# sumitsk/algp

Hardware: AMD Instinct MI355X
Metric: GP-fit+MI-score throughput (N train x M candidates) (higher is better)
Workload: dtype f64

## Files before the change

### algp_amd/csrc/api.hip

```cpp
#include "api_impl.h"

using namespace algp;

namespace algp {

int fail(algp_ctx* c, int code, const std::string& msg) {
    if (c) c->err = msg;
    return code;
}

int ensure(algp_ctx* c, DevBuf& b, size_t bytes) {
    if (bytes <= b.cap && b.p) return ALGP_OK;
    if (bytes == 0) bytes = 256;
    if (b.p) {
        hipStreamSynchronize(c->stream);
        hipFree(b.p);
        c->dev_bytes -= (int64_t)b.cap;
        b.p = nullptr;
        b.cap = 0;
    }
    const size_t want = (bytes + 255) / 256 * 256;
    hipError_t e = hipMalloc(&b.p, want);
    if (e != hipSuccess) {
        b.p = nullptr;
// ... 437 lines not shown

template struct Impl<float>;
template struct Impl<double>;

}

extern "C" {

int algp_version(void) { return 100; }

int algp_device_count(void) {
    int n = 0;
    if (hipGetDeviceCount(&n) != hipSuccess) { (void)hipGetLastError(); return 0; }
    return n;
}

int algp_create(int device_id, int dtype, algp_ctx** out) {
    if (!out || (dtype != ALGP_F32 && dtype != ALGP_F64)) return ALGP_ERR_BAD_ARG;
    *out = nullptr;
    setenv("GPU_MAX_HW_QUEUES", "8", 0);
    int n = 0;
    if (hipGetDeviceCount(&n) != hipSuccess || n <= 0) { (void)hipGetLastError(); return ALGP_ERR_NO_DEVICE; }
    if (device_id < 0 || device_id >= n) return ALGP_ERR_BAD_ARG;
    if (hipSetDevice(device_id) != hipSuccess) return ALGP_ERR_HIP;
    algp_ctx* c = new algp_ctx();
    c->device = device_id;
    c->dtype = dtype;
    c->es = dtype == ALGP_F64 ? 8 : 4;
    if (hipStreamCreateWithFlags(&c->stream, hipStreamNonBlocking) != hipSuccess) { delete c; return ALGP_ERR_HIP; }
    if (hipStreamCreateWithFlags(&c->stream2, hipStreamNonBlocking) != hipSuccess) { hipStreamDestroy(c->stream); delete c; return ALGP_ERR_HIP; }
    if (hipStreamCreateWithFlags(&c->stream3, hipStreamNonBlocking) != hipSuccess) c->stream3 = nullptr;
    if (hipStreamCreateWithFlags(&c->stream4, hipStreamNonBlocking) != hipSuccess) c->stream4 = nullptr;
    c->trsm_chunks = env_int("ALGP_TRSM_CHUNKS", c->trsm_chunks);
    c->cur = c->stream;
    if (ensure(c, c->scal, sizeof(double) * SC_COUNT) != ALGP_OK) { hipStreamDestroy(c->stream); delete c; return ALGP_ERR_OOM; }
    hipMemsetAsync(c->scal.p, 0, sizeof(double) * SC_COUNT, c->stream);
    hipStreamSynchronize(c->stream);
    *out = c;
    return ALGP_OK;
}

void algp_destroy(algp_ctx* c) {
    if (!c) return;
    hipSetDevice(c->device);
    hipStreamSynchronize(c->stream);
    prof_collect(c);
    DevBuf* bufs[] = {&c->Xs, &c->Xraw, &c->Cp, &c->Aidx, &c->yA, &c->varA, &c->y0, &c->L, &c->invD, &c->z, &c->alpha,
                      &c->scal, &c->Cidx, &c->ckind, &c->cextra, &c->Vt, &c->dstat, &c->mu, &c->alive, &c->scores,
                      &c->lrow, &c->remote, &c->commbuf, &c->tvec, &c->amax, &c->prevrows, &c->fresh, &c->lazypicks, &c->yraw, &c->uvec, &c->wvec, &c->acc3, &c->rowstat, &c->inv512, &c->inv512_scr, &c->trsm_tmp, &c->splitk, &c->dag_state, &c->dag_stats, &c->trsv_ctrl, &c->auxA, &c->auxInv, &c->auxW, &c->auxIdx,
                      &c->auxVar, &c->auxD, &c->hostStage, &c->rowx, &c->tailE, &c->tailPart, &c->ldpart};
    for (DevBuf* b : bufs) release(c, *b);
    release(c, c->mi);
    release(c, c->vr);
    dag_release(c);
    comm_destroy(c);
    for (hipEvent_t e : c->event_pool) hipEventDestroy(e);
    for (hipEvent_t e : c->sync_events) hipEventDestroy(e);
    hipStreamSynchronize(c->stream2);
    hipStreamDestroy(c->stream2);
    if (c->stream3) { hipStreamSynchronize(c->stream3); hipStreamDestroy(c->stream3); }
    if (c->stream4) { hipStreamSynchronize(c->stream4); hipStreamDestroy(c->stream4); }
    hipStreamDestroy(c->stream);
    delete c;
}

const char* algp_last_error(const algp_ctx* c) { return c ? c->err.c_str() : "null context"; }

int64_t algp_last_pivot(const algp_ctx* c) { return c ? c->pivot : 0; }

double algp_last_jitter(const algp_ctx* c) { return c ? c->last_jitter : 0.0; }

int algp_dtype(const algp_ctx* c) { return c ? c->dtype : -1; }

int algp_set_hypers(algp_ctx* c, int kernel, int D, const double* log_ls, double log_os, double log_noise) {
    CHECK_CTX(c);
    if (D < 1 || D > MAXD || !log_ls) return fail(c, ALGP_ERR_BAD_ARG, "set_hypers: 1 <= D <= 8 required");
    if (kernel != ALGP_KERNEL_RBF && kernel != ALGP_KERNEL_MATERN15) return fail(c, ALGP_ERR_BAD_ARG, "set_hypers: unknown kernel");
    if (c->hyp.set && c->hyp.D != D && c->n_pool > 0 && !c->pool_is_cov) {
        c->n_pool = 0;
        c->N = 0;
        c->pos_in_train.clear();
    }
// ... 50 lines not shown
    if (N < 0 || (N > 0 && (!idx || !y))) return fail(c, ALGP_ERR_BAD_ARG, "set_train: bad arguments");
    for (int64_t i = 0; i < N; ++i)
        if (idx[i] < 0 || idx[i] >= c->n_pool) return fail(c, ALGP_ERR_BAD_ARG, "set_train: index outside the pool");
    FINISH(c, DISPATCH(c, set_train(c, idx, N, y, var)));
}

int algp_set_constant_mean(algp_ctx* c, int enable, double value) {
    CHECK_CTX(c);
    if (enable && !(value == value)) return fail(c, ALGP_ERR_BAD_ARG, "set_constant_mean: NaN");
    c->mean_override = enable != 0;
    c->mean_value = value;
    return ALGP_OK;
}

#if ALGP_TEST_HOOKS
int64_t algp_debug_counter(algp_ctx* c, int which) {
    if (!c) return -1;
    switch (which) {
        case 0: return c->n_syncs;
        case 1: return c->factor_rows_from_vt;
        case 2: return c->rows_from_peers;
        case 3: return c->row_exchanges;
        case 4: return c->row_fallbacks;
        default: return -1;
    }
}
#endif

#if ALGP_TEST_HOOKS
int algp_debug_set_trsm_chunks(algp_ctx* c, int chunks) {
    CHECK_CTX(c);
    if (chunks < 0 || chunks > 4) return fail(c, ALGP_ERR_BAD_ARG, "debug_set_trsm_chunks: 0 (default) .. 4");
    hipStreamSynchronize(c->stream);
    if (chunks == 0) chunks = env_int("ALGP_TRSM_CHUNKS", 3);
    c->trsm_chunks = chunks;
    return ALGP_OK;
}
#endif

#if ALGP_TEST_HOOKS
int algp_debug_trsv_stall(algp_ctx* c, int block) {
    CHECK_CTX(c);
    if (block < -1) return fail(c, ALGP_ERR_BAD_ARG, "debug_trsv_stall: a block >= 0, or -1 to disarm");
    c->debug_trsv_stall_block = block;
    return ALGP_OK;
}
#endif

#if ALGP_TEST_HOOKS
int algp_debug_dag_stall(algp_ctx* c, int ticket) {
    CHECK_CTX(c);
    if (ticket < -1) return fail(c, ALGP_ERR_BAD_ARG, "debug_dag_stall: a ticket >= 0, or -1 to disarm");
    c->debug_dag_stall_ticket = ticket;
    return ALGP_OK;
}
#endif

int algp_entropy_from_cov(algp_ctx* c, const void* cov, int64_t k, double* H) {
    CHECK_CTX(c);
    if (k < 0 || !H || (k > 0 && !cov)) return fail(c, ALGP_ERR_BAD_ARG, "entropy_from_cov: bad arguments");
    FINISH(c, DISPATCH(c, entropy_from_cov(c, cov, k, H, nullptr, nullptr)));
}

int algp_set_entropy(algp_ctx* c, const int64_t* idx, int64_t m, const void* var, double* H) {
    CHECK_CTX(c);
    NEED_HYPERS(c);
// ... 103 lines not shown
```

### algp_amd/csrc/common.h

```cpp
#pragma once
#include <stdlib.h>
#include <hip/hip_runtime.h>
#include <stdint.h>
#include <string>
#include <vector>
#include "../../include/algp_hip.h"

namespace algp {

constexpr int NB = 128;
constexpr int MAXD = 8;
constexpr int MAX_APPEND = 128;
constexpr double ENT_CONST = 1.4189385332046727;

inline int64_t round_up(int64_t v, int64_t m) { return (v + m - 1) / m * m; }

constexpr int SC_LOGDET = 0;
constexpr int SC_INFO = 1;
constexpr int SC_AUXLOGDET = 2;
constexpr int SC_AUXINFO = 3;
constexpr int SC_AMAXV = 4;
constexpr int SC_AMAXI = 5;
constexpr int SC_PROBE = 6;
constexpr int SC_COMMIT = 8;
// ... 91 lines not shown

namespace algp {
__device__ __forceinline__ float kexp(float x) { return expf(x); }
__device__ __forceinline__ double kexp(double x) {
    const double k = __builtin_rint(x * 1.4426950408889634074);
    double r = __builtin_fma(-k, 6.93147180369123816490e-01, x);
    r = __builtin_fma(-k, 1.90821492927058770002e-10, r);
    double p = 1.6059043836821614599e-10;
    p = __builtin_fma(p, r, 2.0876756987868098979e-09);
    p = __builtin_fma(p, r, 2.5052108385441718775e-08);
    p = __builtin_fma(p, r, 2.7557319223985890653e-07);
    p = __builtin_fma(p, r, 2.7557319223985892511e-06);
    p = __builtin_fma(p, r, 2.4801587301587301566e-05);
    p = __builtin_fma(p, r, 1.9841269841269841253e-04);
    p = __builtin_fma(p, r, 1.3888888888888889419e-03);
    p = __builtin_fma(p, r, 8.3333333333333332177e-03);
    p = __builtin_fma(p, r, 4.1666666666666664354e-02);
    p = __builtin_fma(p, r, 1.6666666666666665741e-01);
    p = __builtin_fma(p, r, 0.5);
    p = __builtin_fma(p, r, 1.0);
    p = __builtin_fma(p, r, 1.0);
    return __builtin_ldexp(p, (int)k);
}
}

struct algp_ctx {
    int device = 0;
    int dtype = ALGP_F64;
    size_t es = 8;
    hipStream_t stream = nullptr;
    hipStream_t stream2 = nullptr;
    hipStream_t stream3 = nullptr, stream4 = nullptr;
    int trsm_chunks = 3;
    hipStream_t cur = nullptr;
    std::vector<hipEvent_t> sync_events;
    std::string err;
    int64_t pivot = 0;
    double last_jitter = 0;
    algp::Hypers hyp;

    int64_t n_pool = 0;
    bool pool_is_cov = false;
    algp::DevBuf Xs;
    algp::DevBuf Xraw;
    algp::DevBuf Cp;
    std::vector<int64_t> pos_in_train;
    std::vector<uint64_t> site_hash;

    int64_t N = 0, Npad = 0;
    int64_t Lld = 0;
    int64_t Nfact = 0;
    std::vector<int64_t> fact_idx;
    std::vector<double> fact_var;
    std::vector<double> train_var_host;
    uint64_t fact_hyp_stamp = 0, hyp_stamp = 1;
    bool train_dirty = false;
    int64_t kept_rows_last = 0;
    std::vector<int64_t> train_idx;
    bool mean_override = false;
    double mean_value = 0;
    bool train_has_repeats = false;
    algp::DevBuf Aidx, yA, varA, y0, L, invD, z, alpha, scal;
    double ybar = 0, logdet = 0, yalpha = 0;
    bool factored = false;
    algp::DevBuf yraw, uvec, wvec;
    std::vector<double> train_y_host, fact_y;
    int64_t uw_rows = 0;
    int64_t uw_stable = 0;
    algp::DevBuf acc3;
    algp::DevBuf rowstat;
    algp::DevBuf splitk;
    algp::DevBuf ldpart;
    algp::DevBuf tailPart;
    algp::DevBuf tailE;
    algp::DevBuf inv512, inv512_scr, trsm_tmp;
    std::vector<algp::DagCache> dag_cache;
    algp::DevBuf dag_state;
    algp::DevBuf trsv_ctrl;
    algp::DevBuf dag_stats;
    int64_t acc_cols = 0, acc_M = -1;
    int64_t factor_rows_from_vt = 0;
    bool alpha_valid = false;

    int64_t M = 0, Mpad = 0, ldv = 0;
    int64_t ncols = 0;
    int prior_noise = 1;
    std::vector<int64_t> cand_idx;
    std::vector<int64_t> cand_pos;
    algp::DevBuf Cidx, ckind, cextra, Vt, dstat, mu, alive, scores, lrow, tvec, amax;
    std::vector<algp::PickRec> picks;
    algp::DevBuf prevrows;
    algp::DevBuf remote;
    algp::DevBuf fresh, lazypicks;
    bool lazy_stale = false;
    bool bounds_valid = false;
    double lazy_ss = 0, lazy_delta = 0;
    bool solved = false;
    int64_t ldv_cap = 0;
    std::vector<int64_t> vt_fact_idx, vt_cand_idx;
    std::vector<double> vt_fact_var;
    std::vector<int> vt_kind;
    uint64_t vt_hyp_stamp = 0;
    int vt_prior_noise = -1;
    bool vt_has_extra = false;
    int64_t kept_cols_last = 0;

    algp::MiState mi;
// ... 187 lines not shown
```

### algp_amd/csrc/gemm.hip

```cpp
#include "common.h"
#include <hip/hip_ext.h>
#include "mfma.h"
#include <algorithm>
#include <type_traits>
#include <stdio.h>
#include <stdlib.h>

namespace algp {

template <typename T>
struct GemmArgs {
    const T* A;
    const T* B;
    const T* C;
    T* D;
    int64_t lda, ldb, ldc, ldd;
    int64_t sA, sB, sC, sD;
    int tiles_m, tiles_n, ktiles;
    T alpha, beta;
    int lower_only;
    int ktri;
    int kcut;
    const T* stat_w;
    T* stat_out;
    int64_t stat_ld;
};

typedef __attribute__((address_space(3))) void* lds_vp;
typedef const __attribute__((address_space(1))) void* glb_vp;

template <int CTRL>
__device__ __forceinline__ float dpp_row(float x) {
    return __int_as_float(__builtin_amdgcn_update_dpp(0, __float_as_int(x), CTRL, 0xf, 0xf, false));
}
template <int CTRL>
__device__ __forceinline__ double dpp_row(double x) {
    const int lo = __builtin_amdgcn_update_dpp(0, __double2loint(x), CTRL, 0xf, 0xf, false);
    const int hi = __builtin_amdgcn_update_dpp(0, __double2hiint(x), CTRL, 0xf, 0xf, false);
    return __hiloint2double(hi, lo);
}
template <typename T>
__device__ __forceinline__ T row16_sum(T x) {
    x += dpp_row<0x128>(x);
    x += dpp_row<0x124>(x);
    x += dpp_row<0x122>(x);
    x += dpp_row<0x121>(x);
    return x;
}

template <typename T>
struct VrGemmArgs : GemmArgs<T> {
    const int64_t* cidx;
    const int* ckind;
    int64_t M;
    int64_t ncol0;
    const T* Xs;
    const T* Cp;
    int64_t n_pool;
// ... 46 lines not shown
                const int col = wc * 64 + j * 16 + fr;
                const int64_t pcol = pc[col];
                T cv;
                if (g.Cp) {
                    cv = g.Cp[prow * g.n_pool + pcol];
                } else {
                    T r2 = (T)0;
#pragma unroll
                    for (int d = 0; d < MAXD; ++d) {
                        const T df = xrow[d] - xc[col * MAXD + d];
                        r2 += df * df;
                    }
                    if (g.kernel == ALGP_KERNEL_RBF) cv = g.os * kexp((T)-0.5 * r2);
                    else {
                        const T rr = sqrt(r2) * (T)1.7320508075688772;
                        cv = g.os * ((T)1 + rr) * kexp(-rr);
                    }
                    if (prow == pcol) cv += g.noise;
                }
                T e = kap * cv - acc[i][j][r];
                e = mc[col] ? e : (T)0;
                s2 += e * e;
            }
            s2 = row16_sum<T>(s2);
            if (fr == 0) red[wc * 128 + row] = s2;
        }
    __syncthreads();
    if (tid < 128) g.stat_out[(int64_t)bn * g.stat_ld + m0 + tid] = red[tid] + red[128 + tid];
}

#ifndef ALGP_GEMM_XOR_MASK
#define ALGP_GEMM_XOR_MASK 2
#endif
template <typename T, bool STATS = false, typename Args = GemmArgs<T>>
__global__ __launch_bounds__(256, 2) void gemm_nt_kernel_dma4(Args g) {
    constexpr bool VR = !std::is_same<Args, GemmArgs<T>>::value;
    static_assert(!(VR && STATS), "one epilogue per kernel");
    constexpr int NST = 4;
    using F = MF<T>;
    using acc_t = typename F::acc_t;
    using chunk_t = typename F::chunk_t;
    constexpr int EPC = F::EPC;
    constexpr int BK = 4 * EPC;

    __shared__ __attribute__((aligned(1024))) char smem[NST * 16384];

    const int nwg = gridDim.x;
    int bm, bn;
    if (g.ktri) {
        int local = blockIdx.x >> 3;
        bm = blockIdx.x & 7;
        while (bm < g.tiles_m && local > bm) { local -= bm + 1; bm += 8; }
        if (bm >= g.tiles_m) return;
        bn = local;
    } else {
        int sid;
        {
            const int id = blockIdx.x, xcd = id & 7, q = nwg >> 3, r = nwg & 7;
            sid = (xcd < r ? xcd * (q + 1) : r * (q + 1) + (xcd - r) * q) + (id >> 3);
        }
        if (g.lower_only) {
            bm = (int)((sqrt(8.0 * (double)sid + 1.0) - 1.0) * 0.5);
            while ((int64_t)(bm + 1) * (bm + 2) / 2 <= sid) ++bm;
            while ((int64_t)bm * (bm + 1) / 2 > sid) --bm;
            bn = sid - (int)((int64_t)bm * (bm + 1) / 2);
        } else {
            bm = sid / g.tiles_n;
            bn = sid - bm * g.tiles_n;
        }
    }
    const int64_t m0 = (int64_t)bm * 128, n0 = (int64_t)bn * 128;
    const int kskip = g.ktri ? bm * (128 / (4 * MF<T>::EPC)) : 0;
    const int tid = threadIdx.x, lane = tid & 63;
    const int wave = __builtin_amdgcn_readfirstlane(tid >> 6);
    const int wr = wave >> 1, wc = wave & 1;
    const int64_t bz = blockIdx.y;

    const int srow = lane >> 2;
    const int schunk = (lane & 3) ^ ((lane >> 4) & ALGP_GEMM_XOR_MASK);
    const T* Ag = g.A + bz * g.sA + (m0 + 32 * wave + srow) * g.lda + schunk * EPC + (int64_t)kskip * BK;
    const T* Bg = g.B + bz * g.sB + (n0 + 32 * wave + srow) * g.ldb + schunk * EPC + (int64_t)kskip * BK;
    auto stage = [&](int st, int kt) {
        char* As = smem + st * 16384 + wave * 2048;
        char* Bs = As + 8192;
#pragma unroll
        for (int i = 0; i < 2; ++i) {
            __builtin_amdgcn_global_load_lds((glb_vp)(Ag + (int64_t)(16 * i) * g.lda + (int64_t)kt * BK),
                                             (lds_vp)(As + i * 1024), 16, 0, 0);
            __builtin_amdgcn_global_load_lds((glb_vp)(Bg + (int64_t)(16 * i) * g.ldb + (int64_t)kt * BK),
                                             (lds_vp)(Bs + i * 1024), 16, 0, 0);
        }
    };

    const int fr = lane & 15, fg = lane >> 4;
    const int coff = ((fg ^ ((fr >> 2) & ALGP_GEMM_XOR_MASK)) << 4);
    const int aoff = (wr * 64 + fr) * 64 + coff;
    const int boff = (wc * 64 + fr) * 64 + coff;

    acc_t acc[4][4];
#pragma unroll
    for (int i = 0; i < 4; ++i)
#pragma unroll
        for (int j = 0; j < 4; ++j)
#pragma unroll
            for (int r = 0; r < 4; ++r) acc[i][j][r] = (T)0;

    int nkt = g.ktiles * 2 - kskip;
    if (g.kcut && (bn + 1) * (128 / BK) < nkt) nkt = (bn + 1) * (128 / BK);
#pragma unroll
    for (int t = 0; t < NST - 1; ++t)
        if (t < nkt) stage(t, t);

    auto fread = [&](int st, chunk_t (&a)[4], chunk_t (&b)[4]) {
        const char* As = smem + st * 16384;
        const char* Bs = As + 8192;
#pragma unroll
        for (int t = 0; t < 4; ++t) a[t] = *reinterpret_cast<const chunk_t*>(As + aoff + t * 1024);
#pragma unroll
        for (int t = 0; t < 4; ++t) b[t] = *reinterpret_cast<const chunk_t*>(Bs + boff + t * 1024);
    };
    auto fmac = [&](const chunk_t (&a)[4], const chunk_t (&b)[4]) {
#pragma unroll
        for (int j = 0; j < 4; ++j)
#pragma unroll
            for (int e = 0; e < EPC; ++e)
#pragma unroll
                for (int i = 0; i < 4; ++i) acc[i][j] = F::mfma(a[i][e], b[j][e], acc[i][j]);
    };
    auto arrive = [&](int younger) {
        if (younger >= 2) __builtin_amdgcn_s_waitcnt(0x0F78);
        else if (younger >= 1) __builtin_amdgcn_s_waitcnt(0x0F74);
        else __builtin_amdgcn_s_waitcnt(0x0F70);
        __builtin_amdgcn_s_barrier();
        asm volatile("" ::: "memory");
    };

    int st = 0;
    for (int kt = 0; kt < nkt; ++kt) {
        arrive(nkt - 1 - kt);
        chunk_t a[4], b[4];
        fread(st, a, b);
        if (kt + NST - 1 < nkt) stage(st == 0 ? NST - 1 : st - 1, kt + NST - 1);
        fmac(a, b);
        st = (st + 1 == NST) ? 0 : st + 1;
    }

    if constexpr (VR) {
        vr_epilogue<T>(g, smem, acc, m0, n0, bn, wr, wc, lane, tid);
        return;
    }
    const T alpha = g.alpha, beta = g.beta;
    const T* Cb = g.C + bz * g.sC;
    T* Db = g.D + bz * g.sD;
    if (beta != (T)0) {
#pragma unroll
        for (int i = 0; i < 4; ++i) {
            T cv[4][4];
#pragma unroll
            for (int r = 0; r < 4; ++r) {
                const int64_t gi = m0 + wr * 64 + i * 16 + F::row_of(lane, r);
#pragma unroll
                for (int j = 0; j < 4; ++j) cv[r][j] = Cb[gi * g.ldc + n0 + wc * 64 + j * 16 + fr];
            }
#pragma unroll
            for (int r = 0; r < 4; ++r) {
                const int64_t gi = m0 + wr * 64 + i * 16 + F::row_of(lane, r);
#pragma unroll
                for (int j = 0; j < 4; ++j)
                    Db[gi * g.ldd + n0 + wc * 64 + j * 16 + fr] = alpha * acc[i][j][r] + beta * cv[r][j];
            }
        }
    } else if (!STATS) {
#pragma unroll
        for (int i = 0; i < 4; ++i)
#pragma unroll
            for (int r = 0; r < 4; ++r) {
                const int64_t gi = m0 + wr * 64 + i * 16 + F::row_of(lane, r);
#pragma unroll
                for (int j = 0; j < 4; ++j) Db[gi * g.ldd + n0 + wc * 64 + j * 16 + fr] = alpha * acc[i][j][r];
            }
    } else {
        T wv[4];
#pragma unroll
        for (int j = 0; j < 4; ++j) wv[j] = g.stat_w[n0 + wc * 64 + j * 16 + fr];
        T* red = reinterpret_cast<T*>(smem);
        __syncthreads();
#pragma unroll
        for (int i = 0; i < 4; ++i)
#pragma unroll
            for (int r = 0; r < 4; ++r) {
                const int row = wr * 64 + i * 16 + F::row_of(lane, r);
                T s2 = (T)0, sw = (T)0;
#pragma unroll
                for (int j = 0; j < 4; ++j) {
                    const T d = alpha * acc[i][j][r];
                    Db[(m0 + row) * g.ldd + n0 + wc * 64 + j * 16 + fr] = d;
                    s2 += d * d;
                    sw += d * wv[j];
                }
                s2 = row16_sum<T>(s2);
                sw = row16_sum<T>(sw);
                if (fr == 0) {
                    red[(wc * 128 + row) * 2 + 0] = s2;
                    red[(wc * 128 + row) * 2 + 1] = sw;
                }
            }
        __syncthreads();
        const int row = tid >> 1, q = tid & 1;
        g.stat_out[(int64_t)(2 * bn + q) * g.stat_ld + m0 + row] = red[row * 2 + q] + red[(128 + row) * 2 + q];
    }
}

static void launch_log_line(int klass, int64_t m, int64_t n, int64_t k, int lower_only, int batch, int ktri, int es, int kcut) {
    static FILE* launch_log = getenv("ALGP_LAUNCH_LOG") ? fopen(getenv("ALGP_LAUNCH_LOG"), "w") : nullptr;
    if (!launch_log) return;
    fprintf(launch_log, "%d %lld %lld %lld %d %d %d %d %d\n", klass, (long long)m, (long long)n, (long long)k, lower_only, batch, ktri, es, kcut);
    fflush(launch_log);
}

template <typename T>
int gemm_nt_launch_batched(algp_ctx* c, int klass, int64_t m, int64_t n, int64_t k, T alpha, const T* A, int64_t lda,
                           int64_t sA, const T* B, int64_t ldb, int64_t sB, T beta, const T* C, int64_t ldc, int64_t sC,
                           T* D, int64_t ldd, int64_t sD, int lower_only, int batch, int ktri, const T* stat_w, T* stat_out,
                           int64_t stat_ld, int kcut) {
    if (m <= 0 || n <= 0 || batch <= 0) return ALGP_OK;
    if (stat_out && (beta != (T)0 || batch != 1 || lower_only || ktri))
        return fail(c, ALGP_ERR_BAD_ARG, "gemm_nt: row statistics need beta = 0, no batch");
    if (kcut && (k != n || lower_only || ktri)) return fail(c, ALGP_ERR_BAD_ARG, "gemm_nt: kcut needs k == n");
    if (m % 128 || n % 128 || k % 128 || k <= 0 || lda % 4 || ldb % 4 || sA % 4 || sB % 4)
        return fail(c, ALGP_ERR_BAD_ARG, "gemm_nt: operands must be padded to multiples of 128");
    if (lower_only && m != n) return fail(c, ALGP_ERR_BAD_ARG, "gemm_nt: lower_only needs a square output");
    if (batch > 65535) return fail(c, ALGP_ERR_BAD_ARG, "gemm_nt: batch too large");
    GemmArgs<T> g;
    g.A = A; g.B = B; g.C = C ? C : D; g.D = D;
    g.lda = lda; g.ldb = ldb; g.ldc = ldc; g.ldd = ldd;
    g.sA = sA; g.sB = sB; g.sC = sC; g.sD = sD;
    g.tiles_m = (int)(m / 128);
    g.tiles_n = (int)(n / 128);
    g.ktiles = (int)(k / (8 * MF<T>::EPC));
    g.alpha = alpha; g.beta = beta;
    g.lower_only = lower_only;
    g.ktri = ktri;
    g.stat_w = stat_w;
    g.stat_out = stat_out;
    g.stat_ld = stat_ld;
    g.kcut = kcut;
    if (ktri && (!lower_only || k != m)) return fail(c, ALGP_ERR_BAD_ARG, "gemm_nt: ktri needs a square lower-only product with k == m");
    const int64_t tiles = lower_only ? (int64_t)g.tiles_m * (g.tiles_m + 1) / 2 : (int64_t)g.tiles_m * g.tiles_n;
    if (tiles > 0x7fffffff) return fail(c, ALGP_ERR_BAD_ARG, "gemm_nt: grid too large");
    const double tm = (double)g.tiles_m;
    const double flops = ktri ? 2.0 * 128.0 * 128.0 * 128.0 * tm * (tm + 1.0) * (tm + 2.0) / 6.0 * batch
                         : kcut ? 2.0 * 128.0 * 128.0 * 128.0 * tm * (double)g.tiles_n * (g.tiles_n + 1.0) / 2.0 * batch
                              : 2.0 * 128.0 * 128.0 * (double)k * (double)tiles * batch;
    const double bytes = sizeof(T) * batch * ((double)tiles * 128.0 * 128.0 * (beta != (T)0 ? 2.0 : 1.0) +
                                              (double)k * 128.0 * (double)(g.tiles_m + g.tiles_n));
    launch_log_line(klass, m, n, k, lower_only, batch, ktri, (int)sizeof(T), kcut);
    int64_t gx = tiles;
    if (ktri) {
        int64_t most = 0;
        for (int x = 0; x < 8; ++x) {
            int64_t cnt = 0;
            for (int64_t r = x; r < g.tiles_m; r += 8) cnt += r + 1;
            most = std::max(most, cnt);
        }
        gx = 8 * most;
    }
    const dim3 grid((unsigned)gx, (unsigned)batch);
    hipEvent_t ev_a, ev_b;
    const bool timed = prof_launch_events(c, klass, flops, bytes, &ev_a, &ev_b);
    if (stat_out) {
        if (timed) hipExtLaunchKernelGGL((gemm_nt_kernel_dma4<T, true>), grid, dim3(256), 0, c->cur, ev_a, ev_b, 0, g);
        else hipLaunchKernelGGL((gemm_nt_kernel_dma4<T, true>), grid, dim3(256), 0, c->cur, g);
    } else {
        if (timed) hipExtLaunchKernelGGL((gemm_nt_kernel_dma4<T, false>), grid, dim3(256), 0, c->cur, ev_a, ev_b, 0, g);
        else hipLaunchKernelGGL((gemm_nt_kernel_dma4<T, false>), grid, dim3(256), 0, c->cur, g);
    }
    ALGP_HIP(hipGetLastError());
    return ALGP_OK;
}

template <typename T>
int gemm_nt_launch_vr(algp_ctx* c, int klass, int64_t mpad, int64_t n, int64_t k, const T* Vt, int64_t ldv, int64_t ncol0,
                      const KmatSrc& s, const int64_t* cidx, const int* ckind, int64_t M, T* part, int64_t part_ld) {
    if (mpad <= 0 || n <= 0) return ALGP_OK;
    if (mpad % 128 || n % 128 || k % 128 || k <= 0 || ldv % 4 || ncol0 % 128 || ncol0 + n > mpad || k > ldv || s.DP > MAXD)
        return fail(c, ALGP_ERR_BAD_ARG, "gemm_nt_vr: operands must be padded to multiples of 128");
    VrGemmArgs<T> g;
    g.A = Vt; g.B = Vt + ncol0 * ldv; g.C = nullptr; g.D = nullptr;
    g.lda = ldv; g.ldb = ldv; g.ldc = 0; g.ldd = 0;
    g.sA = g.sB = g.sC = g.sD = 0;
    g.tiles_m = (int)(mpad / 128);
    g.tiles_n = (int)(n / 128);
    g.ktiles = (int)(k / (8 * MF<T>::EPC));
    g.alpha = (T)1; g.beta = (T)0;
    g.lower_only = 0; g.ktri = 0; g.kcut = 0;
    g.stat_w = nullptr; g.stat_out = part; g.stat_ld = part_ld;
    g.cidx = cidx; g.ckind = ckind; g.M = M; g.ncol0 = ncol0;
    g.Xs = (const T*)s.Xs; g.Cp = (const T*)s.Cp; g.n_pool = s.n_pool; g.DP = s.DP; g.kernel = s.kernel;
    g.os = (T)s.outputscale; g.noise = (T)s.noise;
    const int64_t tiles = (int64_t)g.tiles_m * g.tiles_n;
    if (tiles > 0x7fffffff) return fail(c, ALGP_ERR_BAD_ARG, "gemm_nt_vr: grid too large");
    const double flops = 2.0 * 128.0 * 128.0 * (double)k * (double)tiles;
    const double bytes = sizeof(T) * ((double)k * 128.0 * (double)(g.tiles_m + g.tiles_n) + 128.0 * (double)tiles);
    launch_log_line(klass, mpad, n, k, 0, 1, 0, (int)sizeof(T), 0);
    hipEvent_t ev_a, ev_b;
    const bool timed = prof_launch_events(c, klass, flops, bytes, &ev_a, &ev_b);
    const dim3 grid((unsigned)tiles);
    if (timed) hipExtLaunchKernelGGL((gemm_nt_kernel_dma4<T, false, VrGemmArgs<T>>), grid, dim3(256), 0, c->cur, ev_a, ev_b, 0, g);
    else hipLaunchKernelGGL((gemm_nt_kernel_dma4<T, false, VrGemmArgs<T>>), grid, dim3(256), 0, c->cur, g);
    ALGP_HIP(hipGetLastError());
    return ALGP_OK;
}
template int gemm_nt_launch_vr<double>(algp_ctx*, int, int64_t, int64_t, int64_t, const double*, int64_t, int64_t, const KmatSrc&,
                                       const int64_t*, const int*, int64_t, double*, int64_t);
template int gemm_nt_launch_vr<float>(algp_ctx*, int, int64_t, int64_t, int64_t, const float*, int64_t, int64_t, const KmatSrc&,
                                      const int64_t*, const int*, int64_t, float*, int64_t);

template <typename T>
int gemm_nt_launch(algp_ctx* c, int klass, int64_t m, int64_t n, int64_t k, T alpha, const T* A,
                   int64_t lda, const T* B, int64_t ldb, T beta, const T* C, int64_t ldc, T* D,
                   int64_t ldd, int lower_only) {
    return gemm_nt_launch_batched<T>(c, klass, m, n, k, alpha, A, lda, 0, B, ldb, 0, beta, C, ldc, 0, D, ldd, 0,
                                     lower_only, 1, 0, nullptr, nullptr, 0, 0);
}
template <typename T>
int gemm_nt_launch_stats(algp_ctx* c, int klass, int64_t m, int64_t k, T alpha, const T* A, int64_t lda, const T* B, int64_t ldb,
                         T* D, int64_t ldd, const T* w, T* stat_out, int64_t stat_ld) {
    return gemm_nt_launch_batched<T>(c, klass, m, 128, k, alpha, A, lda, 0, B, ldb, 0, (T)0, nullptr, 0, 0, D, ldd, 0, 0, 1, 0, w,
                                     stat_out, stat_ld, 0);
// ... 48 lines not shown
int test_mfma_launch(algp_ctx* c, int* mismatches_dev) {
    hipLaunchKernelGGL(mfma_probe_kernel<T>, dim3(1), dim3(64), 0, c->cur, mismatches_dev);
    ALGP_HIP(hipGetLastError());
    return ALGP_OK;
}
template int test_mfma_launch<double>(algp_ctx*, int*);
template int test_mfma_launch<float>(algp_ctx*, int*);


template <typename T>
__global__ void fill_random_kernel(T* p, int64_t n, unsigned seed) {
    const int64_t i = (int64_t)blockIdx.x * blockDim.x + threadIdx.x;
    if (i >= n) return;
    unsigned x = (unsigned)(i * 2654435761u) ^ seed;
    x ^= x >> 16; x *= 0x7feb352du; x ^= x >> 15; x *= 0x846ca68bu; x ^= x >> 16;
    p[i] = (T)((int)(x & 0xffff) - 32768) * (T)(1.0 / 32768.0);
}

template <typename T>
int bench_gemm(algp_ctx* c, int64_t m, int64_t n, int64_t k, int lower_only, int beta_one, int reps,
               double* ms_out) {
    DevBuf a, b, cc;
    int rc = ensure(c, a, sizeof(T) * m * k);
    if (rc == ALGP_OK) rc = ensure(c, b, sizeof(T) * n * k);
    if (rc == ALGP_OK) rc = ensure(c, cc, sizeof(T) * m * n);
    if (rc != ALGP_OK) { hipFree(a.p); hipFree(b.p); hipFree(cc.p); return rc; }
    hipLaunchKernelGGL(fill_random_kernel<T>, dim3((unsigned)((m * k + 255) / 256)), dim3(256), 0, c->cur, (T*)a.p, m * k, 1u);
    hipLaunchKernelGGL(fill_random_kernel<T>, dim3((unsigned)((n * k + 255) / 256)), dim3(256), 0, c->cur, (T*)b.p, n * k, 2u);
    hipLaunchKernelGGL(fill_random_kernel<T>, dim3((unsigned)((m * n + 255) / 256)), dim3(256), 0, c->cur, (T*)cc.p, m * n, 3u);
    hipEvent_t e0, e1;
    hipEventCreate(&e0);
    hipEventCreate(&e1);
    const T beta = beta_one ? (T)1 : (T)0;
    for (int w = 0; w < 2 && rc == ALGP_OK; ++w)
        rc = gemm_nt_launch<T>(c, ALGP_PROF_GEMM_OTHER, m, n, k, (T)-1, (const T*)a.p, k, (const T*)b.p, k, beta,
                               (const T*)cc.p, n, (T*)cc.p, n, lower_only);
    hipEventRecord(e0, c->cur);
    for (int r = 0; r < reps && rc == ALGP_OK; ++r)
        rc = gemm_nt_launch<T>(c, ALGP_PROF_GEMM_OTHER, m, n, k, (T)-1, (const T*)a.p, k, (const T*)b.p, k, beta,
                               (const T*)cc.p, n, (T*)cc.p, n, lower_only);
    hipEventRecord(e1, c->cur);
    hipEventSynchronize(e1);
    float ms = 0;
    hipEventElapsedTime(&ms, e0, e1);
    *ms_out = ms / (reps > 0 ? reps : 1);
    hipEventDestroy(e0);
    hipEventDestroy(e1);
    hipFree(a.p); hipFree(b.p); hipFree(cc.p);
    c->dev_bytes -= (int64_t)(a.cap + b.cap + cc.cap);
    return rc;
}
template int bench_gemm<double>(algp_ctx*, int64_t, int64_t, int64_t, int, int, int, double*);
template int bench_gemm<float>(algp_ctx*, int64_t, int64_t, int64_t, int, int, int, double*);

}
```

### algp_amd/csrc/potrf.hip

```cpp
#include "common.h"
#include "mfma.h"
#include "diag.h"
#include "vecops.h"
#include <stdlib.h>

namespace algp {

template <typename T, bool FACTOR>
__global__ __launch_bounds__(256) void potrf_diag_kernel(T* A, int64_t lda, T* inv_out, double* logdet_acc, int* info,
                                                          int64_t block_row0) {
    __shared__ DiagShared<T> sh;
    diag128_run<T, FACTOR>(sh, A, lda, inv_out, logdet_acc, true, info, block_row0);
}

template <typename T>
int potrf_diag_launch(algp_ctx* c, T* A, int64_t lda, T* inv_out, double* logdet_acc, int* info,
                      int64_t block_row0) {
    ProfScope ps(c, ALGP_PROF_POTRF_DIAG, 128.0 * 128.0 * 128.0, sizeof(T) * 3.0 * 128.0 * 128.0);
    hipLaunchKernelGGL((potrf_diag_kernel<T, true>), dim3(1), dim3(256), 0, c->cur, A, lda, inv_out, logdet_acc,
                       info, block_row0);
    ALGP_HIP(hipGetLastError());
    return ALGP_OK;
}
template int potrf_diag_launch<double>(algp_ctx*, double*, int64_t, double*, double*, int*, int64_t);
// ... 320 lines not shown
                                tmp512);
}

static hipEvent_t sync_event(algp_ctx* c, size_t i) {
    while (c->sync_events.size() <= i) {
        hipEvent_t e;
        hipEventCreateWithFlags(&e, hipEventDisableTiming);
        c->sync_events.push_back(e);
    }
    return c->sync_events[i];
}

template <typename T>
int trsm_blocked(algp_ctx* c, int klass, T* X, int64_t mpad, int64_t ldx, const T* L, int64_t npad,
                 int64_t ldl, const T* invD, int64_t col_start, const T* stat_w, T* stat_out, int64_t stat_ld, bool* stats_done) {
    const int64_t tiles = mpad / NB;
    const bool stats = stat_out && stat_w && col_start == 0 && tiles > TRSM_PUSH_TILES;
    if (stats_done) *stats_done = stats;
    if (!stats) stat_out = nullptr;
    const T* inv512 = nullptr;
    T* tmp512 = nullptr;
    {
        const bool on = env_switch("ALGP_TRSM_INV512", true);
        if (on && col_start == 0 && tiles > TRSM_PUSH_TILES && npad / WB >= 1 && c->cur == c->stream &&
            ensure(c, c->inv512, sizeof(T) * (size_t)(npad / WB) * WB * WB) == ALGP_OK &&
            ensure(c, c->inv512_scr, sizeof(T) * inv512_scratch_elems<T>(npad)) == ALGP_OK &&
            ensure(c, c->trsm_tmp, sizeof(T) * (size_t)mpad * WB) == ALGP_OK) {
            ALGP_TRY(build_inv512<T>(c, klass, L, ldl, invD, npad, (T*)c->inv512.p, (T*)c->inv512_scr.p));
            inv512 = (const T*)c->inv512.p;
            tmp512 = (T*)c->trsm_tmp.p;
            ALGP_HIP(hipMemcpy2DAsync(tmp512, sizeof(T) * WB, X, sizeof(T) * ldx, sizeof(T) * WB, (size_t)mpad, hipMemcpyDeviceToDevice, c->cur));
        }
    }
    hipStream_t streams[4] = {c->stream, c->stream2, c->stream3, c->stream4};
    int nch = c->trsm_chunks < 1 ? 1 : (c->trsm_chunks > 4 ? 4 : c->trsm_chunks);
    while (nch > 1 && (!streams[nch - 1] || tiles < 32 * nch)) --nch;
    if (col_start == 0 && tiles <= TRSM_PUSH_TILES) nch = 1;
    if (nch == 1 || c->cur != c->stream)
        return trsm_rows<T>(c, klass, X, mpad, ldx, L, npad, ldl, invD, col_start, true, stat_w, stat_out, stat_ld, inv512, tmp512);
    ALGP_HIP(hipEventRecord(sync_event(c, 0), streams[0]));
    int rc = ALGP_OK;
    int64_t r0 = 0;
    for (int k = nch - 1; k >= 0; --k) {
        const int64_t rows = (k == 0) ? mpad - r0 : (tiles / nch) * NB;
        if (k > 0) ALGP_HIP(hipStreamWaitEvent(streams[k], sync_event(c, 0), 0));
        c->cur = streams[k];
        if (rc == ALGP_OK)
            rc = trsm_rows<T>(c, klass, X + r0 * ldx, rows, ldx, L, npad, ldl, invD, col_start, false, stat_w,
                              stat_out ? stat_out + r0 : nullptr, stat_ld, inv512, tmp512 ? tmp512 + r0 * WB : nullptr);
        r0 += rows;
    }
    c->cur = streams[0];
    for (int k = 1; k < nch; ++k) {
        hipEventRecord(sync_event(c, (size_t)k), streams[k]);
        hipStreamWaitEvent(streams[0], sync_event(c, (size_t)k), 0);
    }
    return rc;
}
template int trsm_blocked<double>(algp_ctx*, int, double*, int64_t, int64_t, const double*, int64_t, int64_t,
                                  const double*, int64_t, const double*, double*, int64_t, bool*);
template int trsm_blocked<float>(algp_ctx*, int, float*, int64_t, int64_t, const float*, int64_t, int64_t,
                                 const float*, int64_t, const float*, float*, int64_t, bool*);

template <typename T>
__global__ void sub_partials_rect_kernel(T* C, int64_t ldc, int64_t m, int64_t n, const T* P, int nchunks) {
    const int64_t i = (int64_t)blockIdx.y * 16 + (threadIdx.x >> 4), j = (int64_t)blockIdx.x * 16 + (threadIdx.x & 15);
// ... 369 lines not shown
```

Before: 612,900.

## Add persistent scheduled GEMM with split-K tail balancing for TRSM updates

Adds a persistent-workgroup schedule for the non-triangular GEMM used inside the blocked TRSM. It launches two workgroups per CU, each looping over several output tiles with a prefetch of the next tile. The leftover tiles of the final partial round are split along K into partial slices that a small finish kernel reduces. When TRSM uses the inverse-512 path and the chunk count was not set explicitly, this replaces the multi-stream row chunking. The aim is to remove the tail-wave imbalance and the cross-stream overhead, at the cost of an extra reduction kernel, a partial buffer, and more complex kernel control flow.

```diff
diff --git a/algp_amd/csrc/api.hip b/algp_amd/csrc/api.hip
--- a/algp_amd/csrc/api.hip
+++ b/algp_amd/csrc/api.hip
@@ -493,6 +493,8 @@
     if (hipStreamCreateWithFlags(&c->stream3, hipStreamNonBlocking) != hipSuccess) c->stream3 = nullptr;
     if (hipStreamCreateWithFlags(&c->stream4, hipStreamNonBlocking) != hipSuccess) c->stream4 = nullptr;
     c->trsm_chunks = env_int("ALGP_TRSM_CHUNKS", c->trsm_chunks);
+    c->trsm_chunks_explicit = env_int("ALGP_TRSM_CHUNKS", 0) != 0;
+    if (hipDeviceGetAttribute(&c->cu_count, hipDeviceAttributeMultiprocessorCount, device_id) != hipSuccess) { (void)hipGetLastError(); c->cu_count = 0; }
     c->cur = c->stream;
     if (ensure(c, c->scal, sizeof(double) * SC_COUNT) != ALGP_OK) { hipStreamDestroy(c->stream); delete c; return ALGP_ERR_OOM; }
     hipMemsetAsync(c->scal.p, 0, sizeof(double) * SC_COUNT, c->stream);
@@ -508,7 +510,7 @@
     prof_collect(c);
     DevBuf* bufs[] = {&c->Xs, &c->Xraw, &c->Cp, &c->Aidx, &c->yA, &c->varA, &c->y0, &c->L, &c->invD, &c->z, &c->alpha,
                       &c->scal, &c->Cidx, &c->ckind, &c->cextra, &c->Vt, &c->dstat, &c->mu, &c->alive, &c->scores,
-                      &c->lrow, &c->remote, &c->commbuf, &c->tvec, &c->amax, &c->prevrows, &c->fresh, &c->lazypicks, &c->yraw, &c->uvec, &c->wvec, &c->acc3, &c->rowstat, &c->inv512, &c->inv512_scr, &c->trsm_tmp, &c->splitk, &c->dag_state, &c->dag_stats, &c->trsv_ctrl, &c->auxA, &c->auxInv, &c->auxW, &c->auxIdx,
+                      &c->lrow, &c->remote, &c->commbuf, &c->tvec, &c->amax, &c->prevrows, &c->fresh, &c->lazypicks, &c->yraw, &c->uvec, &c->wvec, &c->acc3, &c->rowstat, &c->inv512, &c->inv512_scr, &c->trsm_tmp, &c->gemm_part, &c->splitk, &c->dag_state, &c->dag_stats, &c->trsv_ctrl, &c->auxA, &c->auxInv, &c->auxW, &c->auxIdx,
                       &c->auxVar, &c->auxD, &c->hostStage, &c->rowx, &c->tailE, &c->tailPart, &c->ldpart};
     for (DevBuf* b : bufs) release(c, *b);
     release(c, c->mi);
@@ -625,6 +627,7 @@
     CHECK_CTX(c);
     if (chunks < 0 || chunks > 4) return fail(c, ALGP_ERR_BAD_ARG, "debug_set_trsm_chunks: 0 (default) .. 4");
     hipStreamSynchronize(c->stream);
+    c->trsm_chunks_explicit = chunks != 0 || env_int("ALGP_TRSM_CHUNKS", 0) != 0;
     if (chunks == 0) chunks = env_int("ALGP_TRSM_CHUNKS", 3);
     c->trsm_chunks = chunks;
     return ALGP_OK;
diff --git a/algp_amd/csrc/common.h b/algp_amd/csrc/common.h
--- a/algp_amd/csrc/common.h
+++ b/algp_amd/csrc/common.h
@@ -147,6 +147,9 @@
     hipStream_t stream2 = nullptr;
     hipStream_t stream3 = nullptr, stream4 = nullptr;
     int trsm_chunks = 3;
+    bool trsm_chunks_explicit = false;
+    int cu_count = 0;
+    bool gemm_sched = false;
     hipStream_t cur = nullptr;
     std::vector<hipEvent_t> sync_events;
     std::string err;
@@ -188,6 +191,7 @@
     algp::DevBuf ldpart;
     algp::DevBuf tailPart;
     algp::DevBuf tailE;
+    algp::DevBuf gemm_part;
     algp::DevBuf inv512, inv512_scr, trsm_tmp;
     std::vector<algp::DagCache> dag_cache;
     algp::DevBuf dag_state;
diff --git a/algp_amd/csrc/gemm.hip b/algp_amd/csrc/gemm.hip
--- a/algp_amd/csrc/gemm.hip
+++ b/algp_amd/csrc/gemm.hip
@@ -1,6 +1,7 @@
 #include "common.h"
 #include <hip/hip_ext.h>
 #include "mfma.h"
+#include "gemm_sched.h"
 #include <algorithm>
 #include <type_traits>
 #include <stdio.h>
@@ -24,6 +25,8 @@
     const T* stat_w;
     T* stat_out;
     int64_t stat_ld;
+    Sched sch;
+    T* part;
 };
 
 typedef __attribute__((address_space(3))) void* lds_vp;
@@ -136,10 +139,11 @@
 #ifndef ALGP_GEMM_XOR_MASK
 #define ALGP_GEMM_XOR_MASK 2
 #endif
-template <typename T, bool STATS = false, typename Args = GemmArgs<T>>
+template <typename T, bool STATS = false, typename Args = GemmArgs<T>, bool SCHED = false>
 __global__ __launch_bounds__(256, 2) void gemm_nt_kernel_dma4(Args g) {
     constexpr bool VR = !std::is_same<Args, GemmArgs<T>>::value;
     static_assert(!(VR && STATS), "one epilogue per kernel");
+    static_assert(!(VR && SCHED), "the scheduled form serves the sweep's products only");
     constexpr int NST = 4;
     using F = MF<T>;
     using acc_t = typename F::acc_t;
@@ -147,10 +151,22 @@
     constexpr int EPC = F::EPC;
     constexpr int BK = 4 * EPC;
 
-    __shared__ __attribute__((aligned(1024))) char smem[NST * 16384];
+    __shared__ __attribute__((aligned(1024))) char smem[NST * 16384 + (SCHED && STATS ? 4096 : 0)];
 
     const int nwg = gridDim.x;
     int bm, bn;
+    int kskip = 0;
+    int nkt;
+    int slice = -1, nunits = 1, ui = 0;
+    if constexpr (SCHED) {
+        nunits = sched_count(g.sch, blockIdx.x);
+        const SchedUnit u = sched_unit(g.sch, blockIdx.x, 0);
+        bm = u.tile / g.tiles_n;
+        bn = u.tile - bm * g.tiles_n;
+        kskip = u.kb0 * (128 / BK);
+        nkt = (u.kb1 - u.kb0) * (128 / BK);
+        slice = u.slice;
+    } else {
     if (g.ktri) {
         int local = blockIdx.x >> 3;
         bm = blockIdx.x & 7;
@@ -173,8 +189,10 @@
             bn = sid - bm * g.tiles_n;
         }
     }
-    const int64_t m0 = (int64_t)bm * 128, n0 = (int64_t)bn * 128;
-    const int kskip = g.ktri ? bm * (128 / (4 * MF<T>::EPC)) : 0;
+    kskip = g.ktri ? bm * (128 / BK) : 0;
+    nkt = g.ktiles * 2 - kskip;
+    if (g.kcut && (bn + 1) * (128 / BK) < nkt) nkt = (bn + 1) * (128 / BK);
+    }
     const int tid = threadIdx.x, lane = tid & 63;
     const int wave = __builtin_amdgcn_readfirstlane(tid >> 6);
     const int wr = wave >> 1, wc = wave & 1;
@@ -182,8 +200,8 @@
 
     const int srow = lane >> 2;
     const int schunk = (lane & 3) ^ ((lane >> 4) & ALGP_GEMM_XOR_MASK);
-    const T* Ag = g.A + bz * g.sA + (m0 + 32 * wave + srow) * g.lda + schunk * EPC + (int64_t)kskip * BK;
-    const T* Bg = g.B + bz * g.sB + (n0 + 32 * wave + srow) * g.ldb + schunk * EPC + (int64_t)kskip * BK;
+    const T* Ag = g.A + bz * g.sA + ((int64_t)bm * 128 + 32 * wave + srow) * g.lda + schunk * EPC + (int64_t)kskip * BK;
+    const T* Bg = g.B + bz * g.sB + ((int64_t)bn * 128 + 32 * wave + srow) * g.ldb + schunk * EPC + (int64_t)kskip * BK;
     auto stage = [&](int st, int kt) {
         char* As = smem + st * 16384 + wave * 2048;
         char* Bs = As + 8192;
@@ -202,15 +220,6 @@
     const int boff = (wc * 64 + fr) * 64 + coff;
 
     acc_t acc[4][4];
-#pragma unroll
-    for (int i = 0; i < 4; ++i)
-#pragma unroll
-        for (int j = 0; j < 4; ++j)
-#pragma unroll
-            for (int r = 0; r < 4; ++r) acc[i][j][r] = (T)0;
-
-    int nkt = g.ktiles * 2 - kskip;
-    if (g.kcut && (bn + 1) * (128 / BK) < nkt) nkt = (bn + 1) * (128 / BK);
 #pragma unroll
     for (int t = 0; t < NST - 1; ++t)
         if (t < nkt) stage(t, t);
@@ -240,6 +249,13 @@
     };
 
     int st = 0;
+    for (;;) {
+#pragma unroll
+    for (int i = 0; i < 4; ++i)
+#pragma unroll
+        for (int j = 0; j < 4; ++j)
+#pragma unroll
+            for (int r = 0; r < 4; ++r) acc[i][j][r] = (T)0;
     for (int kt = 0; kt < nkt; ++kt) {
         arrive(nkt - 1 - kt);
         chunk_t a[4], b[4];
@@ -248,15 +264,40 @@
         fmac(a, b);
         st = (st + 1 == NST) ? 0 : st + 1;
     }
+    const int64_t m0 = (int64_t)bm * 128, n0 = (int64_t)bn * 128;
+    const int cur_bn = bn, cur_slice = slice;
+    if constexpr (SCHED) {
+        if (++ui < nunits) {
+            const SchedUnit u = sched_unit(g.sch, blockIdx.x, ui);
+            bm = u.tile / g.tiles_n;
+            bn = u.tile - bm * g.tiles_n;
+            nkt = (u.kb1 - u.kb0) * (128 / BK);
+            slice = u.slice;
+            Ag = g.A + ((int64_t)bm * 128 + 32 * wave + srow) * g.lda + schunk * EPC + (int64_t)u.kb0 * 128;
+            Bg = g.B + ((int64_t)bn * 128 + 32 * wave + srow) * g.ldb + schunk * EPC + (int64_t)u.kb0 * 128;
+#pragma unroll
+            for (int t = 0; t < NST - 1; ++t) stage((st + t) & (NST - 1), t);
+        }
+    }
 
     if constexpr (VR) {
-        vr_epilogue<T>(g, smem, acc, m0, n0, bn, wr, wc, lane, tid);
+        vr_epilogue<T>(g, smem, acc, m0, n0, cur_bn, wr, wc, lane, tid);
         return;
     }
     const T alpha = g.alpha, beta = g.beta;
     const T* Cb = g.C + bz * g.sC;
     T* Db = g.D + bz * g.sD;
-    if (beta != (T)0) {
+    if (SCHED && !STATS && cur_slice >= 0) {
+        T* P = g.part + (int64_t)cur_slice * (128 * 128);
+#pragma unroll
+        for (int i = 0; i < 4; ++i)
+#pragma unroll
+            for (int r = 0; r < 4; ++r) {
+                const int row = wr * 64 + i * 16 + F::row_of(lane, r);
+#pragma unroll
+                for (int j = 0; j < 4; ++j) P[row * 128 + wc * 64 + j * 16 + fr] = alpha * acc[i][j][r];
+            }
+    } else if (beta != (T)0) {
 #pragma unroll
         for (int i = 0; i < 4; ++i) {
             T cv[4][4];
@@ -287,8 +328,8 @@
         T wv[4];
 #pragma unroll
         for (int j = 0; j < 4; ++j) wv[j] = g.stat_w[n0 + wc * 64 + j * 16 + fr];
-        T* red = reinterpret_cast<T*>(smem);
-        __syncthreads();
+        T* red = reinterpret_cast<T*>(smem + (SCHED ? NST * 16384 : 0));
+        if constexpr (!SCHED) __syncthreads();
 #pragma unroll
         for (int i = 0; i < 4; ++i)
 #pragma unroll
@@ -309,9 +350,32 @@
                     red[(wc * 128 + row) * 2 + 1] = sw;
                 }
             }
-        __syncthreads();
+        if constexpr (SCHED) {
+            __builtin_amdgcn_s_waitcnt(0xC07F);
+            __builtin_amdgcn_s_barrier();
+            asm volatile("" ::: "memory");
+        } else {
+            __syncthreads();
+        }
         const int row = tid >> 1, q = tid & 1;
-        g.stat_out[(int64_t)(2 * bn + q) * g.stat_ld + m0 + row] = red[row * 2 + q] + red[(128 + row) * 2 + q];
+        g.stat_out[(int64_t)(2 * cur_bn + q) * g.stat_ld + m0 + row] = red[row * 2 + q] + red[(128 + row) * 2 + q];
+    }
+    if constexpr (!SCHED) return;
+    if (ui >= nunits) return;
+    __builtin_amdgcn_s_waitcnt(0x0F70);
+    }
+}
+
+template <typename T>
+__global__ __launch_bounds__(256) void gemm_finish_kernel(const T* part, int S, int tile0, int tiles_n, T beta, const T* C, int64_t ldc,
+                                                          T* D, int64_t ldd) {
+    const int tile = tile0 + blockIdx.x, bm = tile / tiles_n, bn = tile - bm * tiles_n;
+    const T* P = part + (int64_t)blockIdx.x * S * (128 * 128);
+    for (int e = threadIdx.x; e < 128 * 128; e += 256) {
+        const int64_t row = (int64_t)bm * 128 + (e >> 7), col = (int64_t)bn * 128 + (e & 127);
+        T v = beta * C[row * ldc + col];
+        for (int q = 0; q < S; ++q) v += P[(int64_t)q * (128 * 128) + e];
+        D[row * ldd + col] = v;
     }
 }
 
@@ -349,6 +413,8 @@
     g.stat_out = stat_out;
     g.stat_ld = stat_ld;
     g.kcut = kcut;
+    g.sch = Sched();
+    g.part = nullptr;
     if (ktri && (!lower_only || k != m)) return fail(c, ALGP_ERR_BAD_ARG, "gemm_nt: ktri needs a square lower-only product with k == m");
     const int64_t tiles = lower_only ? (int64_t)g.tiles_m * (g.tiles_m + 1) / 2 : (int64_t)g.tiles_m * g.tiles_n;
     if (tiles > 0x7fffffff) return fail(c, ALGP_ERR_BAD_ARG, "gemm_nt: grid too large");
@@ -369,8 +435,36 @@
         }
         gx = 8 * most;
     }
+    hipEvent_t ev_a, ev_b;
+    if (c->gemm_sched && c->cu_count > 0 && !lower_only && !ktri && batch == 1) {
+        const int slots = 2 * c->cu_count;
+        const bool split = beta != (T)0 && !stat_out && !kcut && c->gemm_part.p &&
+                           c->gemm_part.cap >= sizeof(T) * 128 * 128 * (size_t)slots;
+        g.sch = sched_make(slots, g.tiles_m, g.tiles_n, (int)(k / 128), kcut, split ? 1 : 0);
+        g.part = (T*)c->gemm_part.p;
+        const dim3 sgrid((unsigned)g.sch.G);
+        const bool timed = prof_launch_events(c, klass, flops, bytes, &ev_a, &ev_b);
+        if (stat_out) {
+            if (timed) hipExtLaunchKernelGGL((gemm_nt_kernel_dma4<T, true, GemmArgs<T>, true>), sgrid, dim3(256), 0, c->cur, ev_a, ev_b, 0, g);
+            else hipLaunchKernelGGL((gemm_nt_kernel_dma4<T, true, GemmArgs<T>, true>), sgrid, dim3(256), 0, c->cur, g);
+        } else {
+            if (timed) hipExtLaunchKernelGGL((gemm_nt_kernel_dma4<T, false, GemmArgs<T>, true>), sgrid, dim3(256), 0, c->cur, ev_a, ev_b, 0, g);
+            else hipLaunchKernelGGL((gemm_nt_kernel_dma4<T, false, GemmArgs<T>, true>), sgrid, dim3(256), 0, c->cur, g);
+        }
+        ALGP_HIP(hipGetLastError());
+        if (g.sch.S >= 2) {
+            const double fbytes = sizeof(T) * 128.0 * 128.0 * (double)g.sch.left * (g.sch.S + 2.0);
+            const bool ftimed = prof_launch_events(c, klass, 0.0, fbytes, &ev_a, &ev_b);
+            const dim3 fgrid((unsigned)g.sch.left);
+            if (ftimed) hipExtLaunchKernelGGL(gemm_finish_kernel<T>, fgrid, dim3(256), 0, c->cur, ev_a, ev_b, 0, (const T*)g.part, g.sch.S,
+                                              g.sch.full, g.tiles_n, beta, g.C, ldc, D, ldd);
+            else hipLaunchKernelGGL(gemm_finish_kernel<T>, fgrid, dim3(256), 0, c->cur, (const T*)g.part, g.sch.S, g.sch.full, g.tiles_n,
+                                    beta, g.C, ldc, D, ldd);
+            ALGP_HIP(hipGetLastError());
+        }
+        return ALGP_OK;
+    }
     const dim3 grid((unsigned)gx, (unsigned)batch);
-    hipEvent_t ev_a, ev_b;
     const bool timed = prof_launch_events(c, klass, flops, bytes, &ev_a, &ev_b);
     if (stat_out) {
         if (timed) hipExtLaunchKernelGGL((gemm_nt_kernel_dma4<T, true>), grid, dim3(256), 0, c->cur, ev_a, ev_b, 0, g);
@@ -399,6 +493,7 @@
     g.alpha = (T)1; g.beta = (T)0;
     g.lower_only = 0; g.ktri = 0; g.kcut = 0;
     g.stat_w = nullptr; g.stat_out = part; g.stat_ld = part_ld;
+    g.sch = Sched(); g.part = nullptr;
     g.cidx = cidx; g.ckind = ckind; g.M = M; g.ncol0 = ncol0;
     g.Xs = (const T*)s.Xs; g.Cp = (const T*)s.Cp; g.n_pool = s.n_pool; g.DP = s.DP; g.kernel = s.kernel;
     g.os = (T)s.outputscale; g.noise = (T)s.noise;
@@ -513,6 +608,9 @@
     hipEventCreate(&e0);
     hipEventCreate(&e1);
     const T beta = beta_one ? (T)1 : (T)0;
+    const bool sched = !lower_only && c->cu_count > 0 && env_switch("ALGP_TRSM_SCHED", true) &&
+                       ensure(c, c->gemm_part, sizeof(T) * 128 * 128 * 2 * (size_t)c->cu_count) == ALGP_OK;
+    c->gemm_sched = sched;
     for (int w = 0; w < 2 && rc == ALGP_OK; ++w)
         rc = gemm_nt_launch<T>(c, ALGP_PROF_GEMM_OTHER, m, n, k, (T)-1, (const T*)a.p, k, (const T*)b.p, k, beta,
                                (const T*)cc.p, n, (T*)cc.p, n, lower_only);
@@ -521,6 +619,7 @@
         rc = gemm_nt_launch<T>(c, ALGP_PROF_GEMM_OTHER, m, n, k, (T)-1, (const T*)a.p, k, (const T*)b.p, k, beta,
                                (const T*)cc.p, n, (T*)cc.p, n, lower_only);
     hipEventRecord(e1, c->cur);
+    c->gemm_sched = false;
     hipEventSynchronize(e1);
     float ms = 0;
     hipEventElapsedTime(&ms, e0, e1);
diff --git a/algp_amd/csrc/gemm_sched.h b/algp_amd/csrc/gemm_sched.h
--- /dev/null
+++ b/algp_amd/csrc/gemm_sched.h
@@ -0,0 +1,93 @@
+#pragma once
+
+#if defined(__HIPCC__) || defined(__CUDACC__)
+#define ALGP_SCHED_HD __host__ __device__ inline
+#else
+#define ALGP_SCHED_HD inline
+#endif
+
+namespace algp {
+
+struct Sched {
+    int G;
+    int tiles_m, tiles_n, kblocks, kcut;
+    int tiles, rounds, full, left, S;
+};
+
+struct SchedUnit {
+    int tile;
+    int kb0, kb1;
+    int slice;
+};
+
+ALGP_SCHED_HD Sched sched_make(int slots, int tiles_m, int tiles_n, int kblocks, int kcut, int allow_split) {
+    Sched s;
+    s.tiles_m = tiles_m; s.tiles_n = tiles_n; s.kblocks = kblocks; s.kcut = kcut;
+    s.tiles = tiles_m * tiles_n;
+    s.G = s.tiles < slots ? s.tiles : slots;
+    s.rounds = s.G > 0 ? s.tiles / s.G : 0;
+    s.full = s.rounds * s.G;
+    s.left = s.tiles - s.full;
+    s.S = 0;
+    if (kcut) { s.full = s.tiles; s.left = 0; return s; }
+    if (s.left > 0) {
+        s.S = 1;
+        if (allow_split) {
+            s.S = s.G / s.left;
+            if (s.S > kblocks) s.S = kblocks;
+        }
+    }
+    return s;
+}
+
+ALGP_SCHED_HD void sched_group(const Sched& s, int wg, int* before, int* size, int* local) {
+    const int x = wg & 7, q = s.G >> 3, r = s.G & 7;
+    *before = x < r ? x * (q + 1) : r * (q + 1) + (x - r) * q;
+    *size = q + (x < r ? 1 : 0);
+    *local = wg >> 3;
+}
+
+ALGP_SCHED_HD int sched_count(const Sched& s, int wg) {
+    if (s.kcut) return (s.tiles - wg + s.G - 1) / s.G;
+    int extra = 0;
+    if (s.S >= 2) {
+        int before, size, local;
+        sched_group(s, wg, &before, &size, &local);
+        extra = before + local < s.left * s.S ? 1 : 0;
+    } else if (s.S == 1) {
+        extra = wg < s.left ? 1 : 0;
+    }
+    return s.rounds + extra;
+}
+
+ALGP_SCHED_HD SchedUnit sched_unit(const Sched& s, int wg, int i) {
+    SchedUnit u;
+    u.slice = -1;
+    if (s.kcut) {
+        const int d = wg + i * s.G;
+        const int cls = d / s.tiles_m, bm = d - cls * s.tiles_m, bn = s.tiles_n - 1 - cls;
+        u.tile = bm * s.tiles_n + bn;
+        u.kb0 = 0;
+        u.kb1 = bn + 1 < s.kblocks ? bn + 1 : s.kblocks;
+        return u;
+    }
+    int before, size, local;
+    sched_group(s, wg, &before, &size, &local);
+    u.kb0 = 0;
+    u.kb1 = s.kblocks;
+    if (i < s.rounds) {
+        u.tile = s.rounds * before + i * size + local;
+    } else if (s.S >= 2) {
+        const int pos = before + local;
+        const int sl = pos / s.left, j = pos - sl * s.left;
+        u.tile = s.full + j;
+        u.kb0 = (int)((long long)sl * s.kblocks / s.S);
+        u.kb1 = (int)((long long)(sl + 1) * s.kblocks / s.S);
+        u.slice = j * s.S + sl;
+    } else {
+        u.tile = s.full + wg;
+    }
+    return u;
+}
+
+}
diff --git a/algp_amd/csrc/potrf.hip b/algp_amd/csrc/potrf.hip
--- a/algp_amd/csrc/potrf.hip
+++ b/algp_amd/csrc/potrf.hip
@@ -376,6 +376,13 @@
             ALGP_HIP(hipMemcpy2DAsync(tmp512, sizeof(T) * WB, X, sizeof(T) * ldx, sizeof(T) * WB, (size_t)mpad, hipMemcpyDeviceToDevice, c->cur));
         }
     }
+    if (inv512 && !c->trsm_chunks_explicit && c->cu_count > 0 && env_switch("ALGP_TRSM_SCHED", true) &&
+        ensure(c, c->gemm_part, sizeof(T) * 128 * 128 * 2 * (size_t)c->cu_count) == ALGP_OK) {
+        c->gemm_sched = true;
+        const int rc = trsm_rows<T>(c, klass, X, mpad, ldx, L, npad, ldl, invD, col_start, true, stat_w, stat_out, stat_ld, inv512, tmp512);
+        c->gemm_sched = false;
+        return rc;
+    }
     hipStream_t streams[4] = {c->stream, c->stream2, c->stream3, c->stream4};
     int nch = c->trsm_chunks < 1 ? 1 : (c->trsm_chunks > 4 ? 4 : c->trsm_chunks);
     while (nch > 1 && (!streams[nch - 1] || tiles < 32 * nch)) --nch;
```

Result: faster. 625,300 (median of 6 runs) (+2.0%).
